# RookieJunChen/FullSubNet-plus

Hardware: AMD Instinct MI355X
Metric: STFT frames/sec (257-bin, 2 s clips), FullSubNet+ forward (higher is better)
Workload: dtype f32

## Files before the change

### fullsubnet_plus_amd/csrc/fsnp_common.h

```cpp
#pragma once
#include <hip/hip_runtime.h>
#include <math.h>
#include <stdint.h>

#include "../../include/fsnp.h"
#include "../../include/fsnp_debug.h"

namespace fsnp {

struct Dims {
    int B;
    int T;
    int Tp;
    int F;
    int FP;
    int CH;
    int H;
    int NSB;
    int NIN;
    int LA;
    const int* lens = nullptr;
    const int* tpb = nullptr;
};

// ... 77 lines not shown
    const float* w2g;
    const float* c1;
    const float* c2;
    const float* wf;
    const float* bf;
    int NB, N1P, K1P, N2P, K2P;
    int num_cus;
    int dilation[16];
    int gemm_dma;
};

struct TcnBuffers {
    const float* att;
    float* x;
    float* y1;
    float* y2;
    double* gn;
    float* fb;
    float* dbg_tcn0;
};

void launch_tcn(const Dims& d, int fb_act, const TcnWeights& w, const TcnBuffers& buf, hipStream_t s, int branches = 3);
void launch_linear_act(const float* A, int lda, const float* W, int ldw, const float* bias, float* C, int ldc, int K,
                       int N, int B, int Tp, int act, int num_cus, hipStream_t s, long a_utt_stride = 0, int a_cols = 0);
void launch_stft_pad(const float* wav, long wav_stride, float* xp, long xp_stride, int B, int L, int n_fft, hipStream_t s);
void launch_istft_ola(const float* frames, const float* window, float* wav, long wav_stride, int B, int T, int L, int n_fft,
                      hipStream_t s);
void launch_stft_pad_lengths(const float* wav, long wav_stride, float* xp, long xp_stride, int B, const int* samples, int n_fft, hipStream_t s);
void launch_istft_ola_lengths(const float* frames, const float* window, float* wav, long wav_stride, int B, int T, int L, const int* samples,
                              int n_fft, hipStream_t s);
void stft_build_matrices(int n_fft, float* fwd , float* inv ,
                         float* window );

int launch_norm_stage(int norm_type, const float* in, const int64_t strides[4], float* out, int B, int C, int F, int T, hipStream_t s);
void launch_unfold_stage(const float* in, const int64_t strides[4], float* out, int B, int C, int F, int T, int num_neighbor, hipStream_t s);

struct SubbandBuffers {
    const float* att_mag;
    const float* fb;
    const float* refl_w;
    const float* refl_wfb;
    int NFBN;
    double* acc;
    NormMD* md_utt;
    NormMD* md_row;
};
struct RowDesc { int b, f, out_off, valid; };
constexpr int kGnStride = 16;

void launch_subband_stats(const Dims& d, int norm_type, const SubbandBuffers& buf, const RowDesc* rows,
                          int num_slots, hipStream_t s);
struct SbGatherArgs {
    const float* att_mag; int fb_rel, fb_branch_stride;
    const RowDesc* rows; const NormMD* md_utt; const NormMD* md_row;
    float* x; int xstride;
    int num_slots, Tp, FP, F, NSBN, NFBN, NIN;
};
void launch_sb_gather(const SbGatherArgs& a, hipStream_t s);
void launch_sb_scatter(const float* y, int ystride, const RowDesc* rows, float* out, long out_stride_o, int num_slots,
                       int Tp, int LA, int out_channels, hipStream_t s);

struct LstmWeights {
    const float* wpack;
    const float* wpack12;
    const float* wpack_bf[2];
    int ih_bf16;
    const float* wpack_coop[4];
    const float* wpack_coopn;
    const float* wpack16;
    const float* wpack16_bf;
    const float* wpack_gru;
    const float* wpack_hp;
    const float* wpack_hpw;
    int hp_wave;
    const float* wpack_fbv;
    const float* wpack_coopw;
    const float* wgen;
    int gru;
    int waves;
    const float* bias;
    const float* wfc;
    const float* bfc;
    int H, NIN, KX, OUT;
};
struct LstmArgs {
    const float* att_mag;
    const float* fb;
    int fb_rel;
    int fb_branch_stride;
    const RowDesc* rows;
    const NormMD* md_utt;
    const NormMD* md_row;
    const float* dense;
    int dense_stride;
    const NormMD* md_seq;
    float* seq_out;
    int seq_stride;
    float* out;
    long out_stride_o;
    int num_rows;
    int num_tiles;
    int ex;
    int Tp, LA, FP, F, NSBN;
    int NFBN;
    int act;
    unsigned long long* prof;
    float* coop_hx;
    unsigned* coop_bar;
    unsigned* coop_bar2;
    int coop_skew;
    unsigned* coop_err;
    unsigned* coop_abort;
    int coop_units;
    int coop_bar_stride;
    int coop_xcd;
    int coop_own_cu;
    int coop_groups;
    int coop_rows_per_group;
    int coop_corrupt;
    int coop_chaos;
    unsigned long long* clk;
};

struct LstmPlan { int num_tiles, ex, rows_per_slot_tile; };
LstmPlan plan_lstm_tiles(int num_rows, int num_cus);
void launch_lstm(const LstmWeights& w, const LstmArgs& a, hipStream_t s);
void launch_lstm16(const LstmWeights& w, const LstmArgs& a, hipStream_t s);
size_t lstm16_pack_floats(int H, int KX);
size_t lstm16_pack_floats_bf16ih(int H, int KX);
void lstm16_pack_weights_bf16ih(int H, int NIN, int KX, const float* wih0, const float* whh0, const float* wih1, const float* whh1, float* wpack);
void lstm16_pack_weights(int H, int NIN, int KX, const float* wih0, const float* whh0, const float* wih1, const float* whh1, float* wpack);
void launch_gru(const LstmWeights& w, const LstmArgs& a, hipStream_t s);
size_t gru_pack_floats(int H, int KX, int NW);
void gru_pack_weights(int H, int NIN, int KX, int NW, const float* wih0, const float* whh0, const float* wih1,
                      const float* whh1, float* wpack);
void launch_lstm_coop(const LstmWeights& w, const LstmArgs& a, hipStream_t s);
void launch_lstm_coop_seq(const LstmWeights& w, const LstmArgs& a, hipStream_t s);
size_t lstm_coop_pack_floats(int H, int KX, int units);
void lstm_coop_pack_weights(int H, int NIN, int KX, int units, const float* wih0, const float* whh0, const float* wih1,
                            const float* whh1, float* wpack);
size_t lstm_coop_exchange_bytes(int H, int row_tiles);
void launch_lstm_hp(const LstmWeights& w, const LstmArgs& a, hipStream_t s);
bool lstm_hp_available(const LstmWeights& w);
void launch_lstm_hpw(const LstmWeights& w, const LstmArgs& a, hipStream_t s);
bool lstm_hpw_available(const LstmWeights& w);
size_t lstm_hpw_pack_floats(int H, int KX);
void lstm_hpw_pack_weights(int H, int NIN, int KX, const float* wih0, const float* whh0, const float* wih1, const float* whh1, float* out);
size_t lstm_hp_pack_floats(int H, int KX);
void lstm_hp_pack_weights(int H, int NIN, int KX, const float* wih0, const float* whh0, const float* wih1, const float* whh1, float* out);
void launch_lstm_coopw(const LstmWeights& w, const LstmArgs& a, hipStream_t s);
bool lstm_coopw_available(const LstmWeights& w, int units);
int lstm_coopw_occupancy(const LstmWeights& w, int units);
size_t lstm_coopw_pack_floats(int H, int KX);
void lstm_coopw_pack_weights(int H, int NIN, int KX, const float* wih0, const float* whh0, const float* wih1, const float* whh1, float* out);
void launch_lstm_fbv(const LstmWeights& w, const LstmArgs& a, hipStream_t s);
bool lstm_fbv_available(const LstmWeights& w, int batch, int num_cus);
size_t lstm_fbv_pack_floats(int H);
void lstm_fbv_pack_weights(int H, int NIN, const float* wih0, const float* whh0, const float* wih1, const float* whh1, float* out);
void launch_lstm_generic(const LstmWeights& w, const LstmArgs& a, bool seq, hipStream_t s);
size_t lstm_generic_pack_floats(int H, int NIN);
void lstm_generic_pack_weights(int H, int NIN, const float* wih0, const float* whh0, const float* wih1, const float* whh1, float* out);
int lstm_generic_rows_per_group(int H, int NIN, int num_seq, int num_cus);
int lstm_generic_check(int H, int NIN, bool seq);
void launch_lstm_coopn(const LstmWeights& w, const LstmArgs& a, hipStream_t s);
size_t lstm_coopn_pack_floats(int H, int KX);
void lstm_coopn_pack_weights(int H, int NIN, int KX, const float* wih0, const float* whh0, const float* wih1,
// ... 54 lines not shown
```

### fullsubnet_plus_amd/csrc/fsnp_weights.hip

```cpp
#include <algorithm>
#include <cstdlib>
#include <cstring>
#include <string>
#include <vector>

#include "fsnp_handle.h"
#include "weight_watch.h"

namespace fsnp {

static const int kDilations[8] = {1, 2, 5, 9, 1, 2, 5, 9};
static const char* kAtt[3] = {"channel_attention", "channel_attention_real", "channel_attention_imag"};
static const char* kFb[3] = {"fb_model", "fb_model_real", "fb_model_imag"};
static const char* kConvNames[3] = {"smallConv1d", "middleConv1d", "largeConv1d"};

void build_specs(fsnp_handle* h) {
    auto add = [&](const std::string& n, int64_t numel) { h->specs.push_back({n, numel}); };
    const int F = h->F, CH = h->CH, H = h->H, Fr = h->Fr;
    const int att = h->cfg.attention;
    const bool fsn = h->model == FSNP_MODEL_FULLSUBNET;
    if (fsn) {
        const std::string f = "fb_model.sequence_model.";
        const int64_t G = h->NG;
        add(f + "weight_ih_l0", G * CH * F);
        add(f + "weight_hh_l0", G * CH * CH);
        add(f + "bias_ih_l0", G * CH);
        add(f + "bias_hh_l0", G * CH);
        add(f + "weight_ih_l1", G * CH * CH);
        add(f + "weight_hh_l1", G * CH * CH);
        add(f + "bias_ih_l1", G * CH);
        add(f + "bias_hh_l1", G * CH);
        add("fb_model.fc_output_layer.weight", (int64_t)F * CH);
        add("fb_model.fc_output_layer.bias", F);
    }
    for (int a = 0; a < 3 && !fsn; ++a) {
        const std::string p = kAtt[a];
        if (att == FSNP_ATT_TSSE) {
            for (int c = 0; c < 3; ++c) {
                add(p + "." + kConvNames[c] + ".0.weight", (int64_t)F * h->cfg.kersize[c]);
                add(p + "." + kConvNames[c] + ".0.bias", F);
            }
            add(p + ".feature_concate_fc.weight", 3);
            add(p + ".feature_concate_fc.bias", 1);
        }
        if (att == FSNP_ATT_ECA) {
            add(p + ".conv.weight", 3);
        } else {
            add(p + ".fc1.weight", (int64_t)Fr * F);
            add(p + ".fc1.bias", Fr);
            add(p + ".fc2.weight", (int64_t)F * Fr);
            add(p + ".fc2.bias", F);
        }
    }
    for (int b = 0; b < 3 && !fsn; ++b) {
        for (int i = 0; i < h->NB; ++i) {
            const std::string p = std::string(kFb[b]) + ".sequence_model." + std::to_string(i);
            add(p + ".conv1x1.weight", (int64_t)CH * F);
            add(p + ".conv1x1.bias", CH);
            add(p + ".prelu1.weight", 1);
            add(p + ".norm1.weight", CH);
            add(p + ".norm1.bias", CH);
            add(p + ".depthwise_conv.weight", (int64_t)CH * 3);
            add(p + ".depthwise_conv.bias", CH);
            add(p + ".prelu2.weight", 1);
            add(p + ".norm2.weight", CH);
            add(p + ".norm2.bias", CH);
            add(p + ".sconv.weight", (int64_t)F * CH);
            add(p + ".sconv.bias", F);
        }
        add(std::string(kFb[b]) + ".fc_output_layer.weight", (int64_t)F * F);
        add(std::string(kFb[b]) + ".fc_output_layer.bias", F);
    }
    if (h->sb_tcn) {
        for (int i = 0; i < 8; ++i) {
            const std::string p = "sb_model.sequence_model." + std::to_string(i);
            add(p + ".conv1x1.weight", (int64_t)CH * h->NIN);
            add(p + ".conv1x1.bias", CH);
            add(p + ".prelu1.weight", 1);
            add(p + ".norm1.weight", CH);
            add(p + ".norm1.bias", CH);
            add(p + ".depthwise_conv.weight", (int64_t)CH * 3);
            add(p + ".depthwise_conv.bias", CH);
            add(p + ".prelu2.weight", 1);
// ... 290 lines not shown
    size_t o_wpack_hp = 0, o_wpack_hpw = 0;
    if (h->planner.hp_ok) {
        o_wpack_hp = alloc(lstm_hp_pack_floats(H, h->KX));
        lstm_hp_pack_weights(H, h->NIN, h->KX, sbw.wih0.data(), sbw.whh0.data(), sbw.wih1.data(), sbw.whh1.data(), blob.data() + o_wpack_hp);
        o_wpack_hpw = alloc(lstm_hpw_pack_floats(H, h->KX));
        lstm_hpw_pack_weights(H, h->NIN, h->KX, sbw.wih0.data(), sbw.whh0.data(), sbw.wih1.data(), sbw.whh1.data(), blob.data() + o_wpack_hpw);
    }
    size_t o_wpack_coopw = 0;
    if (h->planner.coopw_ok) {
        o_wpack_coopw = alloc(lstm_coopw_pack_floats(H, h->KX));
        lstm_coopw_pack_weights(H, h->NIN, h->KX, sbw.wih0.data(), sbw.whh0.data(), sbw.wih1.data(), sbw.whh1.data(), blob.data() + o_wpack_coopw);
    }
    const size_t o_wpack_coopn = alloc(tuned ? lstm_coopn_pack_floats(H, h->KX) : 0);
    if (tuned)
        lstm_coopn_pack_weights(H, h->NIN, h->KX, sbw.wih0.data(), sbw.whh0.data(), sbw.wih1.data(), sbw.whh1.data(),
                                blob.data() + o_wpack_coopn);
    constexpr int KXF = 264;
    size_t o_fbpack[3] = {0, 0, 0}, o_fbbias = 0, o_fsn_wf = 0, o_fsn_bf = 0, o_fbgen = 0, o_fbv = 0;
    bool have_fbv = false;
    const int fsn_kp = (int)align_up(CH, 16), fsn_np = (int)align_up(F, 384);
    if (fsn) {
        const Rnn4 fbw = expand("fb_model.sequence_model.", CH, F);
        if (h->generic_fb) {
            o_fbgen = alloc(lstm_generic_pack_floats(CH, F));
            lstm_generic_pack_weights(CH, F, fbw.wih0.data(), fbw.whh0.data(), fbw.wih1.data(), fbw.whh1.data(), blob.data() + o_fbgen);
        }
        for (int ui = 0; ui < 3 && !h->generic_fb; ++ui) {
            const int units = 8 << ui;
            o_fbpack[ui] = alloc(lstm_coop_pack_floats(CH, KXF, units));
            lstm_coop_pack_weights(CH, F, KXF, units, fbw.wih0.data(), fbw.whh0.data(), fbw.wih1.data(), fbw.whh1.data(),
                                   blob.data() + o_fbpack[ui]);
        }
        if (!h->generic_fb && !h->gru && CH == 512 && F <= 288) {
            o_fbv = alloc(lstm_fbv_pack_floats(CH));
            lstm_fbv_pack_weights(CH, F, fbw.wih0.data(), fbw.whh0.data(), fbw.wih1.data(), fbw.whh1.data(), blob.data() + o_fbv);
            have_fbv = true;
        }
        o_fbbias = alloc(fbw.bias.size());
        std::copy(fbw.bias.begin(), fbw.bias.end(), blob.begin() + o_fbbias);
        o_fsn_wf = alloc((size_t)fsn_np * fsn_kp);
        const auto& wf = W("fb_model.fc_output_layer.weight");
        for (int n = 0; n < F; ++n)
            for (int k = 0; k < CH; ++k) blob[o_fsn_wf + (size_t)n * fsn_kp + k] = wf[(size_t)n * CH + k];
        o_fsn_bf = alloc(fsn_np);
        const auto& bf = W("fb_model.fc_output_layer.bias");
        std::copy(bf.begin(), bf.end(), blob.begin() + o_fsn_bf);
    }
    const size_t o_lbias = alloc(sbw.bias.size());
    std::copy(sbw.bias.begin(), sbw.bias.end(), blob.begin() + o_lbias);
    const size_t o_wfc = h->sb_tcn ? 0 : put("sb_model.fc_output_layer.weight");
    const size_t o_bfc = h->sb_tcn ? 0 : put("sb_model.fc_output_layer.bias");
    const size_t o_refl = alloc(F), o_reflfb = alloc(F);
    for (int f = 0; f < F; ++f) {
        for (int j = 0; j < h->NSB; ++j) blob[o_refl + reflect_index(f - h->cfg.sb_num_neighbors + j, F)] += 1.0f;
        for (int j = 0; j < 2 * h->cfg.fb_num_neighbors + 1; ++j) blob[o_reflfb + reflect_index(f - h->cfg.fb_num_neighbors + j, F)] += 1.0f;
    }

    FSNP_ON_DEVICE(h);
    if (h->d_weights) { FSNP_HIP_CHECK(hipDeviceSynchronize()); FSNP_HIP_CHECK(hipFree(h->d_weights)); h->d_weights = nullptr; }
    FSNP_HIP_CHECK(hipMalloc(reinterpret_cast<void**>(&h->d_weights), blob.size() * sizeof(float)));
    FSNP_HIP_CHECK(hipMemcpy(h->d_weights, blob.data(), blob.size() * sizeof(float), hipMemcpyHostToDevice));
    const float* d = h->d_weights;
    for (int a = 0; a < 3; ++a) {
        for (int c = 0; c < 3; ++c) { h->fw.conv_w[a][c] = d + o_conv_w[a][c]; h->fw.conv_b[a][c] = d + o_conv_b[a][c]; }
        h->fw.cat_w[a] = d + o_cat_w[a]; h->fw.cat_b[a] = d + o_cat_b[a];
        h->fw.fc1_wT[a] = d + o_fc1w[a]; h->fw.fc1_b[a] = d + o_fc1b[a];
        h->fw.fc2_wT[a] = d + o_fc2w[a]; h->fw.fc2_b[a] = d + o_fc2b[a];
    }
    for (int c = 0; c < 3; ++c) h->fw.ksize[c] = h->cfg.kersize[c];
    h->fw.attention = h->cfg.attention;
    h->fw.subband_num = h->cfg.subband_num > 0 ? h->cfg.subband_num : 1;
    bind_tcn(h->tw, fb_off, d);
    h->lw.wpack = d + o_wpack; h->lw.wpack12 = d + o_wpack12; for (int ui = 0; ui < 4; ++ui) h->lw.wpack_coop[ui] = d + o_wpack_coop[ui];
    h->lw.wpack_coopn = d + o_wpack_coopn;
    h->lw.wpack_hp = d + o_wpack_hp;
    h->lw.wpack_hpw = h->planner.hp_ok ? d + o_wpack_hpw : nullptr;
    h->lw.hp_wave = h->hp_wave;
    h->lw.wpack_coopw = h->planner.coopw_ok ? d + o_wpack_coopw : nullptr;
    h->lw.wpack_gru = d + o_wpack_gru;
    h->lw.wpack16 = d + o_wpack16;
    h->lw.wpack16_bf = have16_bf ? d + o_wpack16_bf : nullptr;
    h->lw.wpack_bf[0] = d + o_wpack_bf[0]; h->lw.wpack_bf[1] = d + o_wpack_bf[1]; h->lw.ih_bf16 = h->ih_bf16; h->lw.waves = h->lstm_waves; h->lw.bias = d + o_lbias; h->lw.wfc = d + o_wfc; h->lw.bfc = d + o_bfc;
    h->lw.H = H; h->lw.NIN = h->NIN; h->lw.KX = h->KX; h->lw.OUT = h->cfg.output_size; h->lw.gru = h->gru;
    h->lw.wgen = d + o_wgen;
    if (h->sb_tcn) bind_tcn(h->sbt, sb_off, d);
    if (fsn) {
        h->fbw = LstmWeights{};
        for (int ui = 0; ui < 3; ++ui) h->fbw.wpack_coop[ui] = d + o_fbpack[ui];
        h->fbw.bias = d + o_fbbias;
        h->fbw.H = CH; h->fbw.NIN = F; h->fbw.KX = KXF; h->fbw.OUT = 0; h->fbw.gru = h->gru;
        h->fbw.wgen = d + o_fbgen;
        h->fbw.wpack_fbv = have_fbv ? d + o_fbv : nullptr;
        h->fsn_wf = d + o_fsn_wf; h->fsn_bf = d + o_fsn_bf; h->fsn_kp = fsn_kp;
    }
    h->d_refl_w = d + o_refl;
    h->d_refl_wfb = d + o_reflfb;
    if (tuned) {
        for (int ui = 0; ui < 4; ++ui) h->planner.occ_ksplit[ui] = std::max(1, lstm_coop_occupancy(h->lw, 8 << ui));
        for (int rpg = 1; rpg <= 2; ++rpg) h->planner.occ_coopn[rpg - 1] = std::max(1, lstm_coopn_occupancy(h->lw, rpg));
    }
    for (int ui = 0; ui < 3 && fsn && !h->generic_fb; ++ui) h->occ_fb[ui] = lstm_coop_seq_occupancy(h->fbw, 8 << ui);
    if (h->generic_sb && lstm_generic_check(h->H, h->NIN, false)) return 2;
    if (h->generic_fb && lstm_generic_check(h->CH, h->F, true)) return 2;
    h->committed = true;
    (void)Fr;
    return 0;
}

}
```

### fullsubnet_plus_amd/csrc/lstm.hip

```cpp
#include <cstring>

#include "fsnp_common.h"
#include "lstm_common.h"

namespace fsnp {

template <int EX>
__host__ __device__ __forceinline__ int e_frag_index(int e, int k) {
    return ((((k >> 3) * 2) + (k & 1)) * EX + e) * 4 + ((k >> 1) & 3);
}

struct WStream {
    __amdgpu_buffer_rsrc_t rsrc;
    int voff;
};
template <int NT>
__device__ __forceinline__ float4 wload(const WStream& ws, int g, int n) {
    const auto v = __builtin_amdgcn_raw_buffer_load_b128(ws.rsrc, ws.voff, (g * NT + n) * 1024, 0);
    return __builtin_bit_cast(float4, v);
}

template <int NT, int EX>
__device__ __forceinline__ void mfma_groups(f32x16 (&acc)[NT], float (&accx)[EX > 0 ? EX : 1][NT], float4 (&b)[NT],
                                            const float4* __restrict__ A, const float4* __restrict__ AE, int ngroups,
                                            const WStream& ws, int& gnext, int groups_total) {
    float4 a = A[0];
    float4 ae[EX > 0 ? EX : 1];
#pragma unroll
    for (int e = 0; e < EX; ++e) ae[e] = AE[e];
    for (int g = 0; g < ngroups; ++g) {
        const int gn = (g + 1 < ngroups ? g + 1 : g);
        const float4 an = A[gn * 64];
        float4 aen[EX > 0 ? EX : 1];
#pragma unroll
        for (int e = 0; e < EX; ++e) aen[e] = AE[gn * 2 * EX + e];
        if constexpr (EX == 0) {
#pragma unroll
            for (int n = 0; n < NT; ++n) {
                acc[n] = __builtin_amdgcn_mfma_f32_32x32x2f32(a.x, b[n].x, acc[n], 0, 0, 0);
                acc[n] = __builtin_amdgcn_mfma_f32_32x32x2f32(a.y, b[n].y, acc[n], 0, 0, 0);
                acc[n] = __builtin_amdgcn_mfma_f32_32x32x2f32(a.z, b[n].z, acc[n], 0, 0, 0);
                acc[n] = __builtin_amdgcn_mfma_f32_32x32x2f32(a.w, b[n].w, acc[n], 0, 0, 0);
                b[n] = wload<NT>(ws, gnext, n);
                __builtin_amdgcn_sched_barrier(0);
            }
        } else {
            constexpr int HALF = NT / 2;
#pragma unroll
            for (int hb = 0; hb < NT; hb += HALF) {
#pragma unroll
                for (int n = hb; n < hb + HALF; ++n) {
                    acc[n] = __builtin_amdgcn_mfma_f32_32x32x2f32(a.x, b[n].x, acc[n], 0, 0, 0);
                    acc[n] = __builtin_amdgcn_mfma_f32_32x32x2f32(a.y, b[n].y, acc[n], 0, 0, 0);
                    acc[n] = __builtin_amdgcn_mfma_f32_32x32x2f32(a.z, b[n].z, acc[n], 0, 0, 0);
                    acc[n] = __builtin_amdgcn_mfma_f32_32x32x2f32(a.w, b[n].w, acc[n], 0, 0, 0);
                }
                __builtin_amdgcn_sched_barrier(0);
#pragma unroll
                for (int n = hb; n < hb + HALF; ++n)
#pragma unroll
                    for (int e = 0; e < EX; ++e) {
                        float v = accx[e][n];
                        v = fmaf(ae[e].x, b[n].x, v);
                        v = fmaf(ae[e].y, b[n].y, v);
                        v = fmaf(ae[e].z, b[n].z, v);
                        accx[e][n] = fmaf(ae[e].w, b[n].w, v);
                    }
                __builtin_amdgcn_sched_barrier(0);
#pragma unroll
                for (int n = hb; n < hb + HALF; ++n) b[n] = wload<NT>(ws, gnext, n);
                __builtin_amdgcn_sched_barrier(0);
            }
        }
        gnext = (gnext + 1 == groups_total) ? 0 : gnext + 1;
        a = an;
#pragma unroll
        for (int e = 0; e < EX; ++e) ae[e] = aen[e];
    }
}

__device__ __forceinline__ unsigned short bf16_bits(float v) {
    const unsigned u = __float_as_uint(v);
    return (unsigned short)((u + 0x7FFFu + ((u >> 16) & 1u)) >> 16);
}
__host__ __device__ __forceinline__ int a_frag_index_bf16(int row, int k) {
    return (((k >> 4) * 64) + (((k >> 3) & 1) * 32) + row) * 8 + (k & 7);
}

template <int ST, int UW, int HBLO = 0>
__device__ __forceinline__ void lstm_cell(f32x16 (&acc)[4 * ST], f32x2 (&c)[ST][8], float* __restrict__ Hs, int wave,
                                          int lane, unsigned short* __restrict__ Hb = nullptr) {
#pragma unroll
    for (int s = 0; s < ST; ++s) {
        const int k = wave * UW + s * 32 + (lane & 31);
        const int kbase = (((k >> 3) * 64) + ((k & 1) * 32)) * 4 + ((k >> 1) & 3);
#pragma unroll
        for (int r = 0; r < 16; r += 2) {
            auto rd = [](float v) {
                if constexpr (ST > 1) { float o; asm("v_accvgpr_read_b32 %0, %1" : "=v"(o) : "a"(v)); return o; }
                else return v;
            };
            const f32x2 h = lstm_cell_pair(f32x2{rd(acc[s][r]), rd(acc[s][r + 1])}, f32x2{rd(acc[ST + s][r]), rd(acc[ST + s][r + 1])},
                                           f32x2{rd(acc[2 * ST + s][r]), rd(acc[2 * ST + s][r + 1])},
                                           f32x2{rd(acc[3 * ST + s][r]), rd(acc[3 * ST + s][r + 1])}, c[s][r >> 1]);
            const int row = (r & 3) + 8 * (r >> 2) + 4 * (lane >> 5);
            Hs[kbase + row * 4] = h.x;
            Hs[kbase + (row + 1) * 4] = h.y;
            if (Hb) {
                const unsigned short hx = bf16_bits(h.x), hy = bf16_bits(h.y);
                Hb[a_frag_index_bf16(row, k)] = hx; Hb[a_frag_index_bf16(row + 1, k)] = hy;
                if constexpr (HBLO > 0) {
                    Hb[HBLO + a_frag_index_bf16(row, k)] = bf16_bits(h.x - __uint_as_float((unsigned)hx << 16));
                    Hb[HBLO + a_frag_index_bf16(row + 1, k)] = bf16_bits(h.y - __uint_as_float((unsigned)hy << 16));
                }
            }
        }
    }
}

using bf16x8 = __attribute__((ext_vector_type(8))) __bf16;
template <int NT, int EX, int ALO>
__device__ __forceinline__ void mfma_groups_bf16(f32x16 (&acc)[NT], float (&accx)[EX > 0 ? EX : 1][NT], float4 (&b)[NT],
                                                 const float4* __restrict__ A, const float4* __restrict__ AE, int nsteps,
                                                 const WStream& ws, int& gnext, int groups_total, int lane) {
    float4 a = A[0], al = A[ALO];
    for (int g = 0; g < nsteps; ++g) {
        const float4 an = A[(g + 1 < nsteps ? g + 1 : g) * 64], aln = A[ALO + (g + 1 < nsteps ? g + 1 : g) * 64];
        float4 he[EX > 0 ? EX : 1][2];
        if constexpr (EX > 0) {
            const int kg = 2 * g + (lane >> 5);
#pragma unroll
            for (int e = 0; e < EX; ++e) { he[e][0] = AE[(kg * 2 + 0) * EX + e]; he[e][1] = AE[(kg * 2 + 1) * EX + e]; }
        }
#pragma unroll
        for (int n = 0; n < NT; ++n) {
            if constexpr (EX > 0) {
                const unsigned w0 = __float_as_uint(b[n].x), w1 = __float_as_uint(b[n].y), w2 = __float_as_uint(b[n].z),
                               w3 = __float_as_uint(b[n].w);
#pragma unroll
                for (int e = 0; e < EX; ++e) {
                    float v = accx[e][n];
                    v = fmaf(he[e][0].x, __uint_as_float(w0 << 16), v);
                    v = fmaf(he[e][1].x, __uint_as_float(w0 & 0xFFFF0000u), v);
                    v = fmaf(he[e][0].y, __uint_as_float(w1 << 16), v);
                    v = fmaf(he[e][1].y, __uint_as_float(w1 & 0xFFFF0000u), v);
                    v = fmaf(he[e][0].z, __uint_as_float(w2 << 16), v);
                    v = fmaf(he[e][1].z, __uint_as_float(w2 & 0xFFFF0000u), v);
                    v = fmaf(he[e][0].w, __uint_as_float(w3 << 16), v);
                    accx[e][n] = fmaf(he[e][1].w, __uint_as_float(w3 & 0xFFFF0000u), v);
                }
            }
            acc[n] = __builtin_amdgcn_mfma_f32_32x32x16_bf16(__builtin_bit_cast(bf16x8, a), __builtin_bit_cast(bf16x8, b[n]),
                                                             acc[n], 0, 0, 0);
            if constexpr (ALO > 0)
                acc[n] = __builtin_amdgcn_mfma_f32_32x32x16_bf16(__builtin_bit_cast(bf16x8, al), __builtin_bit_cast(bf16x8, b[n]),
                                                                 acc[n], 0, 0, 0);
            b[n] = wload<NT>(ws, gnext, n);
            __builtin_amdgcn_sched_barrier(0);
        }
        gnext = (gnext + 1 == groups_total) ? 0 : gnext + 1;
        a = an; al = aln;
    }
}

template <int ST, int UW, int EX, int NT>
__device__ __forceinline__ void lstm_cell_extra(float (&accx)[EX > 0 ? EX : 1][NT], float (&cx)[EX > 0 ? EX : 1][ST],
                                                const float* __restrict__ bias, float* __restrict__ He, int wave,
                                                int lane) {
#pragma unroll
    for (int e = 0; e < EX; ++e)
#pragma unroll
        for (int s = 0; s < ST; ++s) {
            float g4[4];
#pragma unroll
            for (int q = 0; q < 4; ++q) {
                const float v = accx[e][q * ST + s];
                g4[q] = v + __shfl_xor(v, 32) + (bias ? bias[(q * ST + s) * 32] : 0.0f);
            }
            const float cn = fast_sigmoid(g4[1]) * cx[e][s] + fast_sigmoid(g4[0]) * fast_tanh(g4[2]);
            cx[e][s] = cn;
            const float h = fast_sigmoid(g4[3]) * fast_tanh(cn);
            if (lane < 32) He[e_frag_index<EX>(e, wave * UW + s * 32 + lane)] = h;
        }
}

template <int HID, int KX, int OUT, int EX, bool PROF, int NW, bool BF>
__global__ __launch_bounds__(64 * NW) __attribute__((amdgpu_waves_per_eu(NW / 4, NW / 4)))
void lstm2_fc_kernel(LstmWeights w, LstmArgs a) {
    static_assert(OUT == 2, "FC lane mapping assumes output_size == 2");
    static_assert(EX >= 0 && EX <= 4, "at most 4 VALU rows per tile (one FC wave per extra row)");
    static_assert(NW % 4 == 0 && NW >= 4, "whole waves per SIMD");
    constexpr int NTHR = 64 * NW;
    constexpr int UW = HID / NW, ST = UW / 32, NT = 4 * ST;
    static_assert(UW % 32 == 0 && UW * NW == HID, "hidden/NW must be a multiple of 32");
    constexpr int KGX = KX / 8, KGH = HID / 8, KG0 = KGX + KGH;
    constexpr int KSB = HID / 16;
    constexpr int KG1 = BF ? KGH + KSB : 2 * KGH, KGT = KG0 + KG1;
    static_assert(KGH % 4 == 0, "FC k-split");
    static_assert(!BF || HID % 16 == 0, "bf16 k-steps");
    constexpr int RT = 32 + EX;
    constexpr int EXA = EX > 0 ? EX : 1;

    extern __shared__ __attribute__((aligned(16))) unsigned char smem_raw[];
    float4* Xs = reinterpret_cast<float4*>(smem_raw);
    float4* H0s = Xs + KGX * 64;
    float4* H1s = H0s + KGH * 64;
    float4* XEs = H1s + KGH * 64;
    float4* HE0s = XEs + KGX * 2 * EX;
    float4* HE1s = HE0s + KGH * 2 * EX;
    float4* Wfc4 = HE1s + KGH * 2 * EX;
    RowDesc* rows_s = reinterpret_cast<RowDesc*>(Wfc4 + OUT * KGH * 2);
    constexpr int BL = BF ? 1 : 2;
    constexpr bool HILO = BF && EX == 0;
    float* Bs = reinterpret_cast<float*>(rows_s + RT);
    float4* H0b = reinterpret_cast<float4*>(Bs + BL * NW * NT * 32);

    const int tid = threadIdx.x;
    const int lane = tid & 63;
    const int wave = __builtin_amdgcn_readfirstlane(tid >> 6);
    const int slot0 = blockIdx.x * RT;
    const int Tp = a.Tp;

    __shared__ unsigned long long clk_s[2];
    if (a.clk != nullptr && tid == 0) {
        clk_s[1] = __builtin_amdgcn_s_memrealtime();
        clk_s[0] = __builtin_amdgcn_s_memtime();
        if (blockIdx.x == 0) { a.clk[0] = clk_s[0]; a.clk[1] = clk_s[1]; a.clk[4] = 0ull; a.clk[5] = 0ull; a.clk[6] = ~0ull; }
    }

    for (int i = tid; i < (KGX + 2 * KGH) * (64 + 2 * EX); i += NTHR) Xs[i] = make_float4(0.f, 0.f, 0.f, 0.f);
    for (int i = tid; i < OUT * KGH * 2; i += NTHR) {
        const int o = i / (KGH * 2), kg = (i >> 1) % KGH, kh = i & 1;
        const float* wr = w.wfc + (size_t)o * HID + kg * 8 + kh;
        Wfc4[i] = make_float4(wr[0], wr[2], wr[4], wr[6]);
    }
    if (tid < RT) rows_s[tid] = a.rows[slot0 + tid];
    for (int i = tid; i < BL * NW * NT * 32; i += NTHR) {
        const int col = i & 31, n = (i >> 5) % NT, wv = (i / (32 * NT)) % NW, layer = BF ? 1 : i / (32 * NT * NW);
        Bs[i] = w.bias[layer * 4 * HID + (n / ST) * HID + wv * UW + (n % ST) * 32 + col];
    }
    __syncthreads();
    if constexpr (BF) {
        if (tid < 32) reinterpret_cast<float*>(Xs)[a_frag_index(tid, w.NIN)] = 1.0f;
        if (EX > 0 && tid < EX) reinterpret_cast<float*>(XEs)[e_frag_index<EXA>(tid, w.NIN)] = 1.0f;
    }

    const bool dense = a.dense != nullptr;
    const float* __restrict__ gbase = dense ? a.dense : a.att_mag;
    const int gstep = dense ? w.NIN : a.FP;
    auto plan = [&](const RowDesc& rd, int j) -> int {
        if (!rd.valid || j >= w.NIN) return -1;
        if (dense) return rd.b * Tp * w.NIN + j;
        return sb_feature_offset(j, rd.f, rd.b * Tp * a.FP, a.F, a.NSBN, a.NFBN, a.fb_rel, a.fb_branch_stride);
    };
    auto row_md = [&](const RowDesc& rd, int slot, NormMD& md, const NormMD*& md_row) {
        md.m = 0.0f; md.d = 1.0f; md_row = nullptr;
        if (dense || !rd.valid) return;
        if (a.md_row != nullptr) md_row = a.md_row + (size_t)slot * Tp;
        else md = a.md_utt[rd.b];
    };
    constexpr int JSTEP = NTHR / 32, NG = (KX + JSTEP - 1) / JSTEP;
    const int grow = tid & 31;
    int goff[NG], xdst[NG];
    NormMD md; const NormMD* md_row;
    {
        const RowDesc rd = rows_s[grow];
#pragma unroll
        for (int i = 0; i < NG; ++i) {
            const int j = (tid >> 5) + JSTEP * i;
            goff[i] = (j < KX && !(BF && j == w.NIN)) ? plan(rd, j) : -2;
            xdst[i] = a_frag_index(grow, j < KX ? j : 0);
        }
        row_md(rd, slot0 + grow, md, md_row);
    }
// ... 22 lines not shown
        }
    }

    const float* __restrict__ bias_l0 = BF ? nullptr : Bs + ((0 * NW + wave) * NT) * 32 + (lane & 31);
    const float* __restrict__ bias_l1 = Bs + (((BL - 1) * NW + wave) * NT) * 32 + (lane & 31);
    f32x2 c0[ST][8], c1[ST][8];
    float cx0[EXA][ST], cx1[EXA][ST];
#pragma unroll
    for (int s = 0; s < ST; ++s) {
#pragma unroll
        for (int r = 0; r < 8; ++r) { c0[s][r] = f32x2{0.0f, 0.0f}; c1[s][r] = f32x2{0.0f, 0.0f}; }
#pragma unroll
        for (int e = 0; e < EXA; ++e) { cx0[e][s] = 0.0f; cx1[e][s] = 0.0f; }
    }

    WStream ws;
    ws.rsrc = __builtin_amdgcn_make_buffer_rsrc(const_cast<float*>(w.wpack) + (size_t)wave * KGT * NT * 256, 0,
                                                KGT * NT * 1024, 0x00020000);
    ws.voff = lane * 16;
    float4 breg[NT];
#pragma unroll
    for (int n = 0; n < NT; ++n) breg[n] = wload<NT>(ws, 0, n);
    int gnext = 1;
    auto run_groups = [&](f32x16 (&acc_)[NT], float (&accx_)[EXA][NT], const float4* A_, const float4* AE_, int ng) {
        mfma_groups<NT, EX>(acc_, accx_, breg, A_, AE_, ng, ws, gnext, KGT);
    };

    const int fc_row = (wave & 3) * 8 + (lane & 7);
    const int fc_o = (lane >> 3) & 1;
    const int fc_kp = lane >> 4;
    const RowDesc fc_rd = rows_s[fc_row];
    const RowDesc fcx_rd = (EX > 0 && wave < EX) ? rows_s[32 + (wave < EX ? wave : 0)] : RowDesc{0, 0, 0, 0};

    auto fc_store = [&](int t_of_h) {
      if (wave < 4) {
        constexpr int KGP = KGH / 4;
        float sum = 0.0f;
#pragma unroll 4
        for (int kk = 0; kk < KGP; ++kk) {
            const int kg = fc_kp * KGP + kk;
#pragma unroll
            for (int kh = 0; kh < 2; ++kh) {
                const float4 h4 = H1s[kg * 64 + kh * 32 + fc_row];
                const float4 w4 = Wfc4[(fc_o * KGH + kg) * 2 + kh];
                sum += h4.x * w4.x + h4.y * w4.y + h4.z * w4.z + h4.w * w4.w;
            }
        }
        sum += __shfl_xor(sum, 16);
        sum += __shfl_xor(sum, 32);
        if (fc_kp == 0 && fc_rd.valid && t_of_h >= a.LA)
            a.out[(size_t)fc_rd.out_off + (size_t)fc_o * a.out_stride_o + (t_of_h - a.LA)] = apply_act(sum + w.bfc[fc_o], a.act);
      }
        if (EX > 0 && wave < EX) {
            const int o = lane >> 5;
            const float* he = reinterpret_cast<const float*>(HE1s);
            float sx = 0.0f;
#pragma unroll 4
            for (int i = 0; i < HID / 32; ++i) {
                const int k = (lane & 31) + 32 * i;
                sx += he[e_frag_index<EXA>(wave, k)] * w.wfc[o * HID + k];
            }
#pragma unroll
            for (int m = 16; m > 0; m >>= 1) sx += __shfl_xor(sx, m);
            if ((lane & 31) == 0 && fcx_rd.valid && t_of_h >= a.LA)
                a.out[(size_t)fcx_rd.out_off + (size_t)o * a.out_stride_o + (t_of_h - a.LA)] = apply_act(sx + w.bfc[o], a.act);
        }
    };

    const float4* AEx = XEs + (lane >> 5) * EX;
    const float4* AEh0 = HE0s + (lane >> 5) * EX;
    const float4* AEh1 = HE1s + (lane >> 5) * EX;

    __syncthreads();

    unsigned long long* prof = nullptr;
    int prof_stride = 0;
    if constexpr (PROF) {
        const bool rec = blockIdx.x == 0 && tid == 0;
        prof = a.prof + (rec ? 0 : (size_t)Tp * 8 + (size_t)blockIdx.x * 256 + tid);
        prof_stride = rec ? 8 : 0;
    }
#define FSNP_STAMP(i) do { if constexpr (PROF) prof[t * prof_stride + (prof_stride ? (i) : 0)] = __builtin_amdgcn_s_memtime(); } while (0)

    for (int t = 0; t < Tp; ++t) {
        FSNP_STAMP(0);
        float xr[NG], xrx = 0.0f;
        NormMD mdn = md, mdxn = mdx;
        const bool have_next = (t + 1 < Tp);
        if (have_next) {
            if (md_row) mdn = md_row[t + 1];
#pragma unroll
            for (int i = 0; i < NG; ++i) xr[i] = goff[i] >= 0 ? gbase[goff[i] + (t + 1) * gstep] : 0.0f;
            if (havex) {
                if (mdx_row) mdxn = mdx_row[t + 1];
                xrx = goffx >= 0 ? gbase[goffx + (t + 1) * gstep] : 0.0f;
            }
        }

        f32x16 acc[NT];
        float accx[EXA][NT];
#pragma unroll
        for (int n = 0; n < NT; ++n) {
#pragma unroll
            for (int r = 0; r < 16; ++r) acc[n][r] = BF ? 0.0f : bias_l0[n * 32];
#pragma unroll
            for (int e = 0; e < EXA; ++e) accx[e][n] = 0.0f;
        }
        run_groups(acc, accx, Xs + lane, AEx, KG0);
        FSNP_STAMP(1);
        __syncthreads();
        FSNP_STAMP(2);
        lstm_cell<ST, UW, HILO ? KSB * 64 * 8 : 0>(acc, c0, reinterpret_cast<float*>(H0s), wave, lane, BF ? reinterpret_cast<unsigned short*>(H0b) : nullptr);
        if (EX > 0) lstm_cell_extra<ST, UW, EX, NT>(accx, cx0, bias_l0, reinterpret_cast<float*>(HE0s), wave, lane);
        if (have_next) {
#pragma unroll
            for (int i = 0; i < NG; ++i)
                if (goff[i] != -2) Xf[xdst[i]] = goff[i] >= 0 ? (xr[i] - mdn.m) / mdn.d : 0.0f;
            if (havex) XEf[xdstx] = goffx >= 0 ? (xrx - mdxn.m) / mdxn.d : 0.0f;
        }
        if (t > 0) fc_store(t - 1);
        FSNP_STAMP(3);
        __syncthreads();
        FSNP_STAMP(4);
#pragma unroll
        for (int n = 0; n < NT; ++n) {
#pragma unroll
            for (int r = 0; r < 16; ++r) acc[n][r] = bias_l1[n * 32];
#pragma unroll
            for (int e = 0; e < EXA; ++e) accx[e][n] = 0.0f;
        }
        run_groups(acc, accx, H1s + lane, AEh1, KGH);
        if constexpr (BF) mfma_groups_bf16<NT, EX, HILO ? KSB * 64 : 0>(acc, accx, breg, H0b + lane, HE0s, KSB, ws, gnext, KGT, lane);
        else run_groups(acc, accx, H0s + lane, AEh0, KGH);
        FSNP_STAMP(5);
        __syncthreads();
        FSNP_STAMP(6);
        lstm_cell<ST, UW>(acc, c1, reinterpret_cast<float*>(H1s), wave, lane);
        if (EX > 0) lstm_cell_extra<ST, UW, EX, NT>(accx, cx1, bias_l1, reinterpret_cast<float*>(HE1s), wave, lane);
        FSNP_STAMP(7);
    }
#undef FSNP_STAMP
    __syncthreads();
    fc_store(Tp - 1);
    if (a.clk != nullptr && tid == 0) {
        const unsigned long long m1 = __builtin_amdgcn_s_memtime(), r1 = __builtin_amdgcn_s_memrealtime();
        if (blockIdx.x == 0) { a.clk[2] = m1; a.clk[3] = r1; }
        atomicMax(a.clk + 4, r1 - clk_s[1]);
        atomicMax(a.clk + 5, m1 - clk_s[0]);
        atomicMin(a.clk + 6, r1 - clk_s[1]);
    }
}

size_t lstm_pack_floats(int H, int KX, int NW) {
    const int NT = 4 * (H / NW / 32);
    const int KGT = KX / 8 + H / 8 + 2 * (H / 8);
    return (size_t)NW * KGT * NT * 64 * 4;
}

void lstm_pack_weights(int H, int NIN, int KX, int NW, const float* wih0, const float* whh0, const float* wih1,
                       const float* whh1, float* wpack) {
    const int UW = H / NW, ST = UW / 32, NT = 4 * ST;
    const int KGX = KX / 8, KGH = H / 8, KG0 = KGX + KGH, KGT = KG0 + 2 * KGH;
    for (int wv = 0; wv < NW; ++wv)
        for (int g = 0; g < KGT; ++g)
            for (int n = 0; n < NT; ++n)
                for (int lane = 0; lane < 64; ++lane)
                    for (int p = 0; p < 4; ++p) {
                        const int gate = n / ST, s = n % ST;
                        const int wrow = gate * H + wv * UW + s * 32 + (lane & 31);
                        float v = 0.0f;
                        if (g < KG0) {
                            const int k = 8 * g + 2 * p + (lane >> 5);
                            if (k < KX) { if (k < NIN) v = wih0[(size_t)wrow * NIN + k]; }
                            else v = whh0[(size_t)wrow * H + (k - KX)];
                        } else {
                            const int k = 8 * (g - KG0) + 2 * p + (lane >> 5);
                            if (k < H) v = whh1[(size_t)wrow * H + k];
                            else v = wih1[(size_t)wrow * H + (k - H)];
                        }
                        wpack[((((size_t)wv * KGT + g) * NT + n) * 64 + lane) * 4 + p] = v;
                    }
}

size_t lstm_pack_floats_bf16ih(int H, int KX, int NW) {
    const int NT = 4 * (H / NW / 32);
    const int KGT = KX / 8 + H / 8 + H / 8 + H / 16;
    return (size_t)NW * KGT * NT * 64 * 4;
}

static unsigned short host_bf16(float v) {
    unsigned u;
    memcpy(&u, &v, 4);
    return (unsigned short)((u + 0x7FFFu + ((u >> 16) & 1u)) >> 16);
}

void lstm_pack_weights_bf16ih(int H, int NIN, int KX, int NW, const float* wih0, const float* whh0, const float* wih1,
                              const float* whh1, const float* bias0, float* wpack) {
    const int UW = H / NW, ST = UW / 32, NT = 4 * ST;
    const int KGX = KX / 8, KGH = H / 8, KG0 = KGX + KGH, KSB = H / 16, KGT = KG0 + KGH + KSB;
    for (int wv = 0; wv < NW; ++wv)
        for (int g = 0; g < KGT; ++g)
            for (int n = 0; n < NT; ++n)
                for (int lane = 0; lane < 64; ++lane) {
                    const int gate = n / ST, s = n % ST;
                    const int wrow = gate * H + wv * UW + s * 32 + (lane & 31);
                    float* dst = wpack + ((((size_t)wv * KGT + g) * NT + n) * 64 + lane) * 4;
                    if (g < KG0 + KGH) {
                        for (int p = 0; p < 4; ++p) {
                            float v = 0.0f;
                            if (g < KG0) {
                                const int k = 8 * g + 2 * p + (lane >> 5);
                                if (k < KX) { if (k < NIN) v = wih0[(size_t)wrow * NIN + k]; else if (k == NIN) v = bias0[wrow]; }
                                else v = whh0[(size_t)wrow * H + (k - KX)];
                            } else {
                                const int k = 8 * (g - KG0) + 2 * p + (lane >> 5);
                                v = whh1[(size_t)wrow * H + k];
                            }
                            dst[p] = v;
                        }
                    } else {
                        const int ks = g - KG0 - KGH;
                        unsigned short* d16 = reinterpret_cast<unsigned short*>(dst);
                        for (int j = 0; j < 8; ++j) d16[j] = host_bf16(wih1[(size_t)wrow * H + 16 * ks + 8 * (lane >> 5) + j]);
                    }
                }
}

template <int EX, int NW, bool BF, int KX, int HID = 384>
static void launch_lstm_ex(const LstmWeights& w, const LstmArgs& a, hipStream_t s) {
    constexpr int OUT = 2;
    constexpr int KGX = KX / 8, KGH = HID / 8, NT = 4 * (HID / NW / 32);
    const size_t smem = (size_t)(KGX + 2 * KGH) * (64 + 2 * EX) * 16 + (size_t)OUT * KGH * 2 * 16 +
                        (32 + EX) * sizeof(RowDesc) + (size_t)(BF ? 1 : 2) * NW * NT * 32 * 4 + (BF ? (size_t)(EX == 0 ? 2 : 1) * (HID / 16) * 64 * 16 : 0);
    LstmWeights wv = w;
    wv.wpack = BF ? (NW == 12 ? w.wpack_bf[1] : w.wpack_bf[0]) : (NW == 12 ? w.wpack12 : w.wpack);
    if constexpr (KX == 40 && HID == 384) {
        if (a.prof != nullptr) {
            auto kern = lstm2_fc_kernel<HID, KX, OUT, EX, true, NW, BF>;
            (void)hipFuncSetAttribute(reinterpret_cast<const void*>(kern), hipFuncAttributeMaxDynamicSharedMemorySize, (int)smem);
            hipLaunchKernelGGL(kern, dim3(a.num_tiles), dim3(64 * NW), smem, s, wv, a);
            return;
        }
    }
    auto kern = lstm2_fc_kernel<HID, KX, OUT, EX, false, NW, BF>;
    static PerDeviceOnce attr_once;
    attr_once.run([&] { (void)hipFuncSetAttribute(reinterpret_cast<const void*>(kern), hipFuncAttributeMaxDynamicSharedMemorySize, (int)smem); });
    hipLaunchKernelGGL(kern, dim3(a.num_tiles), dim3(64 * NW), smem, s, wv, a);
}

template <int NW, bool BF, int KX>
static void launch_lstm_nw(const LstmWeights& w, const LstmArgs& a, hipStream_t s) {
    switch (a.ex) {
        case 0: launch_lstm_ex<0, NW, BF, KX>(w, a, s); break;
        case 1: launch_lstm_ex<1, NW, BF, KX>(w, a, s); break;
        case 2: launch_lstm_ex<2, NW, BF, KX>(w, a, s); break;
        default: launch_lstm_ex<4, NW, BF, KX>(w, a, s); break;
    }
}

void launch_lstm(const LstmWeights& w, const LstmArgs& a, hipStream_t s) {
    if (a.num_tiles <= 0) return;
    const int waves = w.waves != 0 ? w.waves : (a.ex > 0 ? 12 : 4);
    if (w.H == 256) {
        if (w.KX == 64) launch_lstm_ex<0, 4, false, 64, 256>(w, a, s);
        else launch_lstm_ex<0, 4, false, 40, 256>(w, a, s);
        return;
    }
    if (w.KX == 64) {
        if (waves == 12) launch_lstm_nw<12, false, 64>(w, a, s);
        else launch_lstm_nw<4, false, 64>(w, a, s);
    } else if (w.ih_bf16) {
        if (waves == 12) launch_lstm_nw<12, true, 40>(w, a, s);
        else launch_lstm_nw<4, true, 40>(w, a, s);
    } else {
        if (waves == 12) launch_lstm_nw<12, false, 40>(w, a, s);
        else launch_lstm_nw<4, false, 40>(w, a, s);
    }
}

LstmPlan plan_lstm_tiles(int num_rows, int num_cus) {
    LstmPlan p{};
    if (num_rows <= 32 * num_cus) {
        p.ex = 0; p.num_tiles = cdiv(num_rows, 32);
    } else {
        const int cand[4] = {0, 1, 2, 4};
        int best_rounds = 1 << 30;
        for (int i = 0; i < 4; ++i) {
            const int rounds = cdiv(cdiv(num_rows, 32 + cand[i]), num_cus);
            if (rounds < best_rounds) { best_rounds = rounds; p.ex = cand[i]; }
        }
        p.num_tiles = best_rounds * num_cus;
    }
    p.rows_per_slot_tile = 32 + p.ex;
    return p;
}

}
```

Before: 147,000.

## Skip recurrent matmuls at zero state and trim padded x k-pairs

Specializes the first LSTM timestep so the hidden-state matmuls are skipped when the initial state is zero, guarded by a host check that the recurrent weights are finite. It also narrows the input-segment MFMA loop to only the live k-pairs (XP template), dropping MFMAs on zero padding in the x segment. This adds template instantiations and weight-stream refill bookkeeping (gnext/gafter) that must stay consistent, and it increases code size.

```diff
diff --git a/fullsubnet_plus_amd/csrc/fsnp_common.h b/fullsubnet_plus_amd/csrc/fsnp_common.h
--- a/fullsubnet_plus_amd/csrc/fsnp_common.h
+++ b/fullsubnet_plus_amd/csrc/fsnp_common.h
@@ -183,6 +183,7 @@
     const float* wfc;
     const float* bfc;
     int H, NIN, KX, OUT;
+    int zero_state_skip;
 };
 struct LstmArgs {
     const float* att_mag;
diff --git a/fullsubnet_plus_amd/csrc/fsnp_weights.hip b/fullsubnet_plus_amd/csrc/fsnp_weights.hip
--- a/fullsubnet_plus_amd/csrc/fsnp_weights.hip
+++ b/fullsubnet_plus_amd/csrc/fsnp_weights.hip
@@ -1,4 +1,5 @@
 #include <algorithm>
+#include <cmath>
 #include <cstdlib>
 #include <cstring>
 #include <string>
@@ -455,6 +456,10 @@
     h->lw.wpack16_bf = have16_bf ? d + o_wpack16_bf : nullptr;
     h->lw.wpack_bf[0] = d + o_wpack_bf[0]; h->lw.wpack_bf[1] = d + o_wpack_bf[1]; h->lw.ih_bf16 = h->ih_bf16; h->lw.waves = h->lstm_waves; h->lw.bias = d + o_lbias; h->lw.wfc = d + o_wfc; h->lw.bfc = d + o_bfc;
     h->lw.H = H; h->lw.NIN = h->NIN; h->lw.KX = h->KX; h->lw.OUT = h->cfg.output_size; h->lw.gru = h->gru;
+    {
+        auto finite = [](const std::vector<float>& v) { return std::all_of(v.begin(), v.end(), [](float x) { return std::isfinite(x); }); };
+        h->lw.zero_state_skip = finite(sbw.whh0) && finite(sbw.whh1) ? 1 : 0;
+    }
     h->lw.wgen = d + o_wgen;
     if (h->sb_tcn) bind_tcn(h->sbt, sb_off, d);
     if (fsn) {
diff --git a/fullsubnet_plus_amd/csrc/lstm.hip b/fullsubnet_plus_amd/csrc/lstm.hip
--- a/fullsubnet_plus_amd/csrc/lstm.hip
+++ b/fullsubnet_plus_amd/csrc/lstm.hip
@@ -1,4 +1,5 @@
 #include <cstring>
+#include <type_traits>
 
 #include "fsnp_common.h"
 #include "lstm_common.h"
@@ -20,6 +21,51 @@
     return __builtin_bit_cast(float4, v);
 }
 
+template <int NT, int EX, int NP>
+__device__ __forceinline__ void mfma_group(f32x16 (&acc)[NT], float (&accx)[EX > 0 ? EX : 1][NT], float4 (&b)[NT], const float4& a,
+                                           const float4 (&ae)[EX > 0 ? EX : 1], const WStream& ws, int grefill) {
+    static_assert(NP >= 1 && NP <= 4, "live k-pairs per group");
+    if constexpr (EX == 0) {
+#pragma unroll
+        for (int n = 0; n < NT; ++n) {
+            acc[n] = __builtin_amdgcn_mfma_f32_32x32x2f32(a.x, b[n].x, acc[n], 0, 0, 0);
+            if constexpr (NP > 1) acc[n] = __builtin_amdgcn_mfma_f32_32x32x2f32(a.y, b[n].y, acc[n], 0, 0, 0);
+            if constexpr (NP > 2) acc[n] = __builtin_amdgcn_mfma_f32_32x32x2f32(a.z, b[n].z, acc[n], 0, 0, 0);
+            if constexpr (NP > 3) acc[n] = __builtin_amdgcn_mfma_f32_32x32x2f32(a.w, b[n].w, acc[n], 0, 0, 0);
+            b[n] = wload<NT>(ws, grefill, n);
+            __builtin_amdgcn_sched_barrier(0);
+        }
+    } else {
+        constexpr int HALF = NT / 2;
+#pragma unroll
+        for (int hb = 0; hb < NT; hb += HALF) {
+#pragma unroll
+            for (int n = hb; n < hb + HALF; ++n) {
+                acc[n] = __builtin_amdgcn_mfma_f32_32x32x2f32(a.x, b[n].x, acc[n], 0, 0, 0);
+                if constexpr (NP > 1) acc[n] = __builtin_amdgcn_mfma_f32_32x32x2f32(a.y, b[n].y, acc[n], 0, 0, 0);
+                if constexpr (NP > 2) acc[n] = __builtin_amdgcn_mfma_f32_32x32x2f32(a.z, b[n].z, acc[n], 0, 0, 0);
+                if constexpr (NP > 3) acc[n] = __builtin_amdgcn_mfma_f32_32x32x2f32(a.w, b[n].w, acc[n], 0, 0, 0);
+            }
+            __builtin_amdgcn_sched_barrier(0);
+#pragma unroll
+            for (int n = hb; n < hb + HALF; ++n)
+#pragma unroll
+                for (int e = 0; e < EX; ++e) {
+                    float v = accx[e][n];
+                    v = fmaf(ae[e].x, b[n].x, v);
+                    if constexpr (NP > 1) v = fmaf(ae[e].y, b[n].y, v);
+                    if constexpr (NP > 2) v = fmaf(ae[e].z, b[n].z, v);
+                    if constexpr (NP > 3) v = fmaf(ae[e].w, b[n].w, v);
+                    accx[e][n] = v;
+                }
+            __builtin_amdgcn_sched_barrier(0);
+#pragma unroll
+            for (int n = hb; n < hb + HALF; ++n) b[n] = wload<NT>(ws, grefill, n);
+            __builtin_amdgcn_sched_barrier(0);
+        }
+    }
+}
+
 template <int NT, int EX>
 __device__ __forceinline__ void mfma_groups(f32x16 (&acc)[NT], float (&accx)[EX > 0 ? EX : 1][NT], float4 (&b)[NT],
                                             const float4* __restrict__ A, const float4* __restrict__ AE, int ngroups,
@@ -34,49 +80,34 @@
         float4 aen[EX > 0 ? EX : 1];
 #pragma unroll
         for (int e = 0; e < EX; ++e) aen[e] = AE[gn * 2 * EX + e];
-        if constexpr (EX == 0) {
-#pragma unroll
-            for (int n = 0; n < NT; ++n) {
-                acc[n] = __builtin_amdgcn_mfma_f32_32x32x2f32(a.x, b[n].x, acc[n], 0, 0, 0);
-                acc[n] = __builtin_amdgcn_mfma_f32_32x32x2f32(a.y, b[n].y, acc[n], 0, 0, 0);
-                acc[n] = __builtin_amdgcn_mfma_f32_32x32x2f32(a.z, b[n].z, acc[n], 0, 0, 0);
-                acc[n] = __builtin_amdgcn_mfma_f32_32x32x2f32(a.w, b[n].w, acc[n], 0, 0, 0);
-                b[n] = wload<NT>(ws, gnext, n);
-                __builtin_amdgcn_sched_barrier(0);
-            }
-        } else {
-            constexpr int HALF = NT / 2;
-#pragma unroll
-            for (int hb = 0; hb < NT; hb += HALF) {
-#pragma unroll
-                for (int n = hb; n < hb + HALF; ++n) {
-                    acc[n] = __builtin_amdgcn_mfma_f32_32x32x2f32(a.x, b[n].x, acc[n], 0, 0, 0);
-                    acc[n] = __builtin_amdgcn_mfma_f32_32x32x2f32(a.y, b[n].y, acc[n], 0, 0, 0);
-                    acc[n] = __builtin_amdgcn_mfma_f32_32x32x2f32(a.z, b[n].z, acc[n], 0, 0, 0);
-                    acc[n] = __builtin_amdgcn_mfma_f32_32x32x2f32(a.w, b[n].w, acc[n], 0, 0, 0);
-                }
-                __builtin_amdgcn_sched_barrier(0);
-#pragma unroll
-                for (int n = hb; n < hb + HALF; ++n)
-#pragma unroll
-                    for (int e = 0; e < EX; ++e) {
-                        float v = accx[e][n];
-                        v = fmaf(ae[e].x, b[n].x, v);
-                        v = fmaf(ae[e].y, b[n].y, v);
-                        v = fmaf(ae[e].z, b[n].z, v);
-                        accx[e][n] = fmaf(ae[e].w, b[n].w, v);
-                    }
-                __builtin_amdgcn_sched_barrier(0);
-#pragma unroll
-                for (int n = hb; n < hb + HALF; ++n) b[n] = wload<NT>(ws, gnext, n);
-                __builtin_amdgcn_sched_barrier(0);
-            }
-        }
+        mfma_group<NT, EX, 4>(acc, accx, b, a, ae, ws, gnext);
         gnext = (gnext + 1 == groups_total) ? 0 : gnext + 1;
         a = an;
 #pragma unroll
         for (int e = 0; e < EX; ++e) ae[e] = aen[e];
     }
+}
+
+template <int NT, int EX, int XP>
+__device__ __forceinline__ void mfma_x_groups(f32x16 (&acc)[NT], float (&accx)[EX > 0 ? EX : 1][NT], float4 (&b)[NT],
+                                              const float4* __restrict__ A, const float4* __restrict__ AE, const WStream& ws, int gafter) {
+    constexpr int NFULL = XP / 4, REM = XP % 4, NLIVE = NFULL + (REM > 0 ? 1 : 0);
+    float4 a = A[0];
+    float4 ae[EX > 0 ? EX : 1];
+#pragma unroll
+    for (int e = 0; e < EX; ++e) ae[e] = AE[e];
+#pragma unroll
+    for (int g = 0; g < NFULL; ++g) {
+        const float4 an = A[(g + 1) * 64];
+        float4 aen[EX > 0 ? EX : 1];
+#pragma unroll
+        for (int e = 0; e < EX; ++e) aen[e] = AE[(g + 1) * 2 * EX + e];
+        mfma_group<NT, EX, 4>(acc, accx, b, a, ae, ws, g + 1 < NLIVE ? g + 1 : gafter);
+        a = an;
+#pragma unroll
+        for (int e = 0; e < EX; ++e) ae[e] = aen[e];
+    }
+    if constexpr (REM > 0) mfma_group<NT, EX, REM>(acc, accx, b, a, ae, ws, gafter);
 }
 
 __device__ __forceinline__ unsigned short bf16_bits(float v) {
@@ -184,12 +215,13 @@
         }
 }
 
-template <int HID, int KX, int OUT, int EX, bool PROF, int NW, bool BF>
+template <int HID, int KX, int OUT, int EX, bool PROF, int NW, bool BF, int XP>
 __global__ __launch_bounds__(64 * NW) __attribute__((amdgpu_waves_per_eu(NW / 4, NW / 4)))
 void lstm2_fc_kernel(LstmWeights w, LstmArgs a) {
     static_assert(OUT == 2, "FC lane mapping assumes output_size == 2");
     static_assert(EX >= 0 && EX <= 4, "at most 4 VALU rows per tile (one FC wave per extra row)");
     static_assert(NW % 4 == 0 && NW >= 4, "whole waves per SIMD");
+    static_assert(XP >= 1 && 2 * XP <= KX, "live k-pairs of the x segment");
     constexpr int NTHR = 64 * NW;
     constexpr int UW = HID / NW, ST = UW / 32, NT = 4 * ST;
     static_assert(UW % 32 == 0 && UW * NW == HID, "hidden/NW must be a multiple of 32");
@@ -378,7 +410,8 @@
     }
 #define FSNP_STAMP(i) do { if constexpr (PROF) prof[t * prof_stride + (prof_stride ? (i) : 0)] = __builtin_amdgcn_s_memtime(); } while (0)
 
-    for (int t = 0; t < Tp; ++t) {
+    auto step = [&](int t, auto zero_tag) __attribute__((always_inline)) {
+        constexpr bool ZERO = decltype(zero_tag)::value;
         FSNP_STAMP(0);
         float xr[NG], xrx = 0.0f;
         NormMD mdn = md, mdxn = mdx;
@@ -402,7 +435,12 @@
 #pragma unroll
             for (int e = 0; e < EXA; ++e) accx[e][n] = 0.0f;
         }
-        run_groups(acc, accx, Xs + lane, AEx, KG0);
+        {
+            constexpr int gafter = ZERO ? KG0 + KGH : KGX;
+            mfma_x_groups<NT, EX, XP>(acc, accx, breg, Xs + lane, AEx, ws, gafter);
+            gnext = gafter + 1;
+        }
+        if constexpr (!ZERO) run_groups(acc, accx, H0s + lane, AEh0, KGH);
         FSNP_STAMP(1);
         __syncthreads();
         FSNP_STAMP(2);
@@ -425,7 +463,7 @@
 #pragma unroll
             for (int e = 0; e < EXA; ++e) accx[e][n] = 0.0f;
         }
-        run_groups(acc, accx, H1s + lane, AEh1, KGH);
+        if constexpr (!ZERO) run_groups(acc, accx, H1s + lane, AEh1, KGH);
         if constexpr (BF) mfma_groups_bf16<NT, EX, HILO ? KSB * 64 : 0>(acc, accx, breg, H0b + lane, HE0s, KSB, ws, gnext, KGT, lane);
         else run_groups(acc, accx, H0s + lane, AEh0, KGH);
         FSNP_STAMP(5);
@@ -434,7 +472,10 @@
         lstm_cell<ST, UW>(acc, c1, reinterpret_cast<float*>(H1s), wave, lane);
         if (EX > 0) lstm_cell_extra<ST, UW, EX, NT>(accx, cx1, bias_l1, reinterpret_cast<float*>(HE1s), wave, lane);
         FSNP_STAMP(7);
-    }
+    };
+    int t0 = 0;
+    if (Tp > 0 && w.zero_state_skip) { step(0, std::true_type{}); t0 = 1; }
+    for (int t = t0; t < Tp; ++t) step(t, std::false_type{});
 #undef FSNP_STAMP
     __syncthreads();
     fc_store(Tp - 1);
@@ -522,26 +563,36 @@
                 }
 }
 
-template <int EX, int NW, bool BF, int KX, int HID = 384>
-static void launch_lstm_ex(const LstmWeights& w, const LstmArgs& a, hipStream_t s) {
+template <int EX, int NW, bool BF, int KX, int HID, int XP>
+static void launch_lstm_xp(const LstmWeights& w, const LstmArgs& a, hipStream_t s) {
     constexpr int OUT = 2;
     constexpr int KGX = KX / 8, KGH = HID / 8, NT = 4 * (HID / NW / 32);
     const size_t smem = (size_t)(KGX + 2 * KGH) * (64 + 2 * EX) * 16 + (size_t)OUT * KGH * 2 * 16 +
                         (32 + EX) * sizeof(RowDesc) + (size_t)(BF ? 1 : 2) * NW * NT * 32 * 4 + (BF ? (size_t)(EX == 0 ? 2 : 1) * (HID / 16) * 64 * 16 : 0);
     LstmWeights wv = w;
     wv.wpack = BF ? (NW == 12 ? w.wpack_bf[1] : w.wpack_bf[0]) : (NW == 12 ? w.wpack12 : w.wpack);
-    if constexpr (KX == 40 && HID == 384) {
+    if constexpr (KX == 40 && HID == 384 && XP < KX / 2) {
         if (a.prof != nullptr) {
-            auto kern = lstm2_fc_kernel<HID, KX, OUT, EX, true, NW, BF>;
+            auto kern = lstm2_fc_kernel<HID, KX, OUT, EX, true, NW, BF, XP>;
             (void)hipFuncSetAttribute(reinterpret_cast<const void*>(kern), hipFuncAttributeMaxDynamicSharedMemorySize, (int)smem);
             hipLaunchKernelGGL(kern, dim3(a.num_tiles), dim3(64 * NW), smem, s, wv, a);
             return;
         }
     }
-    auto kern = lstm2_fc_kernel<HID, KX, OUT, EX, false, NW, BF>;
+    auto kern = lstm2_fc_kernel<HID, KX, OUT, EX, false, NW, BF, XP>;
     static PerDeviceOnce attr_once;
     attr_once.run([&] { (void)hipFuncSetAttribute(reinterpret_cast<const void*>(kern), hipFuncAttributeMaxDynamicSharedMemorySize, (int)smem); });
     hipLaunchKernelGGL(kern, dim3(a.num_tiles), dim3(64 * NW), smem, s, wv, a);
+}
+
+template <int KX, bool BF>
+constexpr int narrow_x_pairs() { return KX == 40 ? (BF ? 18 : 17) : 26; }
+
+template <int EX, int NW, bool BF, int KX, int HID = 384>
+static void launch_lstm_ex(const LstmWeights& w, const LstmArgs& a, hipStream_t s) {
+    constexpr int XPN = narrow_x_pairs<KX, BF>();
+    if ((w.NIN + (BF ? 1 : 0) + 1) / 2 <= XPN) launch_lstm_xp<EX, NW, BF, KX, HID, XPN>(w, a, s);
+    else launch_lstm_xp<EX, NW, BF, KX, HID, KX / 2>(w, a, s);
 }
 
 template <int NW, bool BF, int KX>
```

Result: no change. 147,600, median of 6 (+0.4%).
